# mnigm2001/Software-Defined-Radio

Hardware: AMD Instinct MI355X
Metric: I/Q MS/s through front-end FIR+decimate+demod(+audio) per job; % HBM roofline (higher is better)
Workload: dtype i8+f32

## Files before the change

### include/fmrx.h

```cpp
#ifndef FMRX_H
#define FMRX_H

#include <stddef.h>
#include <stdint.h>

#ifdef __cplusplus
extern "C" {
#endif

#if defined(__GNUC__)
#define FMRX_API __attribute__((visibility("default")))
#else
#define FMRX_API
#endif

typedef enum fmrx_status {
    FMRX_OK = 0,
    FMRX_EINVAL = 1,
    FMRX_ENODEV = 2,
    FMRX_EHIP = 3,
    FMRX_ENOMEM = 4
} fmrx_status;

FMRX_API const char *fmrx_version(void);
// ... 31 lines not shown
    size_t nseg;
    unsigned repaired;
    float max_dphase, max_dinteg;
    float tol_phase, tol_integ;
} fmrx_pll_parallel_info;
#define FMRX_PLL_RECORD_FLOATS 9
#define fmrx_pll_parallel_max_segments(n) ((size_t)(n) / 32 + 2)
FMRX_API int fmrx_fm_pll_parallel(const float *in, size_t n, float *nco_out, float *state, float freq, float Fs,
                                  float ncoScale, float phaseAdjust, float normBandwidth, double off_hint,
                                  fmrx_pll_parallel_info *info, float *records, uint64_t *mask);
FMRX_API int fmrx_stereo_mix(const float *stereo_filt, const float *pll, size_t n, float *mixer);
FMRX_API int fmrx_stereo_combine(const float *stereo_final, const float *mono, size_t n, float *left, float *right);
FMRX_API int fmrx_pcm16(const float *audio, size_t n, int16_t *out, int wrap);

FMRX_API int fmrx_deemph_design(double fs, double tau_us, float *p, float *b0);
FMRX_API int fmrx_deemph(float *y, const float *x, size_t rows, size_t n, size_t pitch, float p, float b0, float *state,
                         unsigned *missed);
FMRX_API int fmrx_deemph_dev(float *d_y, const float *d_x, size_t rows, size_t n, size_t pitch, float p, float b0, float *d_state,
                             unsigned long long *d_missed, void *stream);

FMRX_API int fmrx_diag_libm(int fn, const float *a, const float *b, size_t n, float *out);
FMRX_API int fmrx_diag_demod_fast(float *out, const float *iq, size_t n, float prev_i, float prev_q, int bounded);
FMRX_API int fmrx_diag_stream_read_dev(const void *d_buf, size_t bytes, int method, void *stream);
FMRX_API int fmrx_estimate_psd(float *freq, float *psd, const float *samples, size_t n, float Fs, int nfft);

typedef struct fmrx_params {
    int mode;
    int rf_Fs, if_Fs;
    float audio_Fs;
    int rf_decim, audio_decim, audio_upsamp;
    int rf_taps;
    int audio_taps;
    int stereo_taps;
    int block_bytes;
} fmrx_params;

FMRX_API int fmrx_mode_params(int mode, int rf_taps, int base_audio_taps, int stereo_taps, fmrx_params *p);

typedef struct fmrx_pipeline fmrx_pipeline;

#define FMRX_PCM_WRAP 1
#define FMRX_PCM_SATURATE 0

FMRX_API int fmrx_pipeline_create(fmrx_pipeline **out, const fmrx_params *p, int channels, size_t max_block_bytes,
                                  int device);
FMRX_API int fmrx_pipeline_destroy(fmrx_pipeline *pl);
// ... 366 lines not shown
```

### software-defined-radio_amd/__init__.py

```python
from __future__ import annotations

import ctypes as C
import os

import numpy as np

_HERE = os.path.dirname(os.path.abspath(__file__))
LIB_PATH = os.environ.get("FMRX_LIB") or os.path.join(_HERE, "lib", "libfmrx.so")
HEADER_PATH = os.path.join(os.path.dirname(_HERE), "include", "fmrx.h")

OK, EINVAL, ENODEV, EHIP, ENOMEM = 0, 1, 2, 3, 4
PCM_WRAP, PCM_SATURATE = 1, 0
TAPS = {"if_i": 0, "if_q": 1, "demod": 2, "mono_filt": 3, "carrier_filt": 4, "stereo_filt": 5, "pll": 6, "mixer": 7,
        "stereo_final": 8, "trig_arg": 9}


class FmrxError(RuntimeError):
    def __init__(self, code: int, msg: str):
        super().__init__(f"fmrx error {code}: {msg}")
        self.code = code


if not os.path.exists(LIB_PATH):
    raise ImportError(
# ... 216 lines not shown


def _option_value(name: str, value) -> int:
    names = _OPTION_NAMES.get(name, {})
    if isinstance(value, str) and value not in names:
        raise FmrxError(EINVAL, f"option {name}: '{value}' is not one of its named values {sorted(names)}")
    return names[value] if isinstance(value, str) else int(value)


def set_option(name: str, value) -> None:
    _check(lib.fmrx_set_option(name.encode(), _option_value(name, value)))


def get_option(name: str) -> int:
    v = C.c_long(0)
    _check(lib.fmrx_get_option(name.encode(), C.byref(v)))
    return v.value


def diagStreamRead(d_ptr, n_bytes, method=0, stream=None) -> None:
    _check(lib.fmrx_diag_stream_read_dev(d_ptr, n_bytes, method, stream))


def hostAlloc(nbytes: int, dtype=np.uint8) -> np.ndarray:
    p = _vp()
    _check(lib.fmrx_host_alloc(C.byref(p), int(nbytes)))
    buf = (C.c_uint8 * int(nbytes)).from_address(p.value)
    arr = np.frombuffer(buf, dtype=dtype)
    arr.flags.writeable = True
    _PINNED[arr.ctypes.data] = (p.value, buf)
    return arr


def hostFree(arr: np.ndarray) -> None:
    p, _ = _PINNED.pop(arr.ctypes.data)
    _check(lib.fmrx_host_free(p))


_PINNED: dict = {}


def deviceLibm(fn: str, a, b=None, flat=False) -> np.ndarray:
    a = _f32(a)
    out = np.zeros(len(a), np.float32)
    bb = _f32(b) if b is not None else None
    _check(lib.fmrx_diag_libm({"sinf": 0, "cosf": 1, "atan2f": 2}[fn] + (3 if flat else 0), a,
# ... 1185 lines not shown
```

### software-defined-radio_amd/csrc/capi.hip

```cpp
#include "fmrx_internal.hpp"
#include "rds_station.hpp"
#include <vector>

#include "build_id.hpp"

namespace fmrx {

static thread_local char g_err[512] = "";

int fail(int code, const char *fmt, ...)
{
    va_list ap;
    va_start(ap, fmt);
    vsnprintf(g_err, sizeof(g_err), fmt, ap);
    va_end(ap);
    return code;
}

int require_device()
{
    int n = 0;
    hipError_t e = hipGetDeviceCount(&n);
    if (e != hipSuccess || n <= 0) {
        (void)hipGetLastError();
// ... 502 lines not shown
    if ((!out || !iq) && n) return fail(FMRX_EINVAL, "diag_demod_fast: null buffer");
    if (bounded != 0 && bounded != 1) return fail(FMRX_EINVAL, "diag_demod_fast: bounded must be 0 or 1");
    if (n == 0) return FMRX_OK;
    FMRX_TRY(require_device());
    Stage st;
    Dev<float> dz, dp, dc;
    const float prev[2] = {prev_i, prev_q};
    FMRX_TRY(st.in(dz, iq, 2 * n));
    FMRX_TRY(st.in(dp, prev, 2));
    FMRX_TRY(st.out(dc, n));
    FMRX_TRY(k_fm_demod_if(dz.p, n, dp.p, nullptr, dc.p, bounded ? 2 : 1, nullptr));
    return st.back(out, dc);
}

int fmrx_diag_stream_read_dev(const void *d_buf, size_t bytes, int method, void *stream)
{
    if (!d_buf || method < 0 || (method & ~0x10000) > 4096) return fail(FMRX_EINVAL, "diag_stream_read_dev: bad arguments");
    FMRX_TRY(require_device());
    Dev<unsigned> sink;
    FMRX_TRY(Stage(kStreamReadSlot, 1).out(sink, 4));
    return k_stream_read(d_buf, bytes, method, sink.p, static_cast<hipStream_t>(stream));
}

int fmrx_estimate_psd(float *freq, float *psd, const float *samples, size_t n, float Fs, int nfft)
{
    if (!freq || !psd || !samples) return fail(FMRX_EINVAL, "estimate_psd: null buffer");
    if (nfft < 2 || nfft % 2 || nfft > 65536) return fail(FMRX_EINVAL, "estimate_psd: nfft must be even and in 2..65536");
    if (n < static_cast<size_t>(nfft)) return fail(FMRX_EINVAL, "estimate_psd: %zu samples < nfft %d", n, nfft);
    if (!(Fs > 0)) return fail(FMRX_EINVAL, "estimate_psd: Fs must be positive");
    FMRX_TRY(require_device());
    Stage st;
    Dev<float> a, b, c, d;
    const size_t nseg = n / nfft, half = nfft / 2;
    FMRX_TRY(st.out(a, n));
    FMRX_TRY(st.put(a.p, samples, nseg * nfft));
    FMRX_TRY(st.out(b, nseg * half));
    FMRX_TRY(st.out(c, half));
    FMRX_TRY(st.out(d, half));
    FMRX_TRY(k_estimate_psd(a.p, n, Fs, nfft, b.p, c.p, d.p, nullptr));
    FMRX_TRY(st.back(freq, c));
    return st.back(psd, d);
}

struct fmrx_fe_plan {
    FePlan plan;
};
// ... 191 lines not shown
```

### software-defined-radio_amd/csrc/fmrx_internal.hpp

```cpp
#pragma once
#include <hip/hip_runtime.h>

#include <cstdarg>
#include <cstdint>
#include <cstdio>
#include <cstdlib>
#include <cstring>
#include <mutex>
#include <string>
#include <vector>

#include "fmrx.h"

namespace fmrx {

int fail(int code, const char *fmt, ...);

#define FMRX_HIP(expr)                                                                         \
    do {                                                                                       \
        hipError_t e_ = (expr);                                                                \
        if (e_ != hipSuccess)                                                                  \
            return ::fmrx::fail(FMRX_EHIP, "%s failed: %s (%s:%d)", #expr, hipGetErrorString(e_), \
                                __FILE__, __LINE__);                                           \
    } while (0)

#define FMRX_TRY(expr)              \
    do {                            \
        int rc_ = (expr);           \
        if (rc_ != FMRX_OK) return rc_; \
    } while (0)

#define FMRX_LAUNCH_CHECK(name, ...)                                                                                              \
    do {                                                                                                                          \
        hipError_t e_ = hipGetLastError();                                                                                        \
        if (e_ != hipSuccess) return ::fmrx::fail(FMRX_EHIP, "launch " name ": %s", ##__VA_ARGS__, hipGetErrorString(e_));        \
    } while (0)

int require_device();

struct Options {
    int fe_variant = 0, tuner_variant = 0, demod = 0, overlap_calls = 0;
    long fused_min_audio = 65536;
    int resample_l2 = 0, resample_exact = 0, resample_chains = 0;
    int pll_warmup = -1, pll_segment = -1, pll_start = 1, pll_mode = 0;
    int deemph_warmup = -1, deemph_segment = -1, deemph_mode = 0;
};
Options &default_options();
std::mutex &options_mutex();
Options options_snapshot();
int set_option_in(Options &o, const char *name, long value);
int get_option_in(const Options &o, const char *name, long *value);

template <typename T>
struct DevBuf {
    T *p = nullptr;
    size_t n = 0;
    DevBuf() = default;
    DevBuf(const DevBuf &) = delete;
    DevBuf &operator=(const DevBuf &) = delete;
    ~DevBuf() { release(); }
    void release()
    {
        if (p) (void)hipFree(p);
        p = nullptr;
        n = 0;
// ... 33 lines not shown
int fe_mfma_bank_lead(const FePlan &pl);
int fe_mfma_bank_launch(const FePlan &pl, const uint8_t *d_slots, long total_bytes, long in_pitch, long block_off, int n_channels,
                        long k_lo, long k_hi, float *d_demod, long out_pitch, long out_off, hipStream_t stream);
int fe_launch(const FePlan &pl, const uint8_t *d_iq, size_t n_samples, const uint8_t *d_hist, float *d_if,
              const Options &o, hipStream_t stream, bool force_generic);
int fe_hist_bytes(int taps, int decim);
bool fe_fused_available(const FePlan &pl, const uint8_t *d_iq, size_t n_samples);
int fe_demod_launch(const FePlan &pl, const uint8_t *d_iq, size_t n_samples, const uint8_t *d_hist,
                    const float *d_prev_override, float *d_demod, float *d_if, float *d_prev_out,
                    uint8_t *d_hist_next, const Options &o, hipStream_t stream);

struct AudioPlan {
    int taps = 0, decim = 0;
    bool fast = false;
    DevBuf<float> table;
    DevBuf<float> h;
    DevBuf<float> mfma_table;
};
int audio_mfma_table_init(AudioPlan &pl, const float *h, int taps, int decim);
bool mono_fused_available(const FePlan &fe, const AudioPlan &au, const uint8_t *d_iq, size_t n_samples, const uint8_t *d_hist);
int mono_fused_launch(const FePlan &fe, const AudioPlan &au, const uint8_t *d_iq, size_t n_samples, const uint8_t *d_hist,
                      const float *d_prev, const float *d_dhist_end, float *d_demod_tail, int tail_keep, float *d_prev_out,
                      float *d_audio, int16_t *d_pcm, int wrap, uint8_t *d_hist_next, const Options &o, hipStream_t stream);
int audio_plan_init(AudioPlan &pl, const float *h, int taps, int decim);
bool audio_fast_available(const AudioPlan &pl, const float *d_x);
int audio_fir_launch(const AudioPlan &pl, const float *d_x, const float *d_hist_end, size_t n_in, int delay, float *d_y,
                     int16_t *d_pcm, int wrap, hipStream_t stream, bool force_generic);

struct ResamplePlan {
    int taps = 0, decim = 0, upsamp = 0;
    int J = 0, JP = 0;
    int span = 0;
    bool fast = false;
    int npass = 0, W = 0, span_l = 0;
    DevBuf<float> table;
    DevBuf<float> h;
    bool mfma = false;
    int mfma_ks4 = 0, mfma_ngroups = 0, mfma_pieces = 0;
    bool mfma_reach_ok = false;
    mutable int mfma_wgs_per_cu[2] = {0, 0};
    DevBuf<float> mfma_img;
    DevBuf<int> mfma_top, mfma_groups;
};
int resample_plan_init(ResamplePlan &pl, const float *h, int taps, int decim, int upsamp);
constexpr int kResampleFront = 256, kResampleBack = 1024;
int resample_launch(const ResamplePlan &pl, const float *d_x, size_t n_in, int delay, float *d_y, const Options &o,
// ... 210 lines not shown
```

### software-defined-radio_amd/csrc/kernels_fe_mfma.hip

```cpp
#include "device_math.hpp"
#include "fe_mfma_host.hpp"
#include "fmrx_internal.hpp"

#include <cmath>
#include <type_traits>
#include <utility>

namespace fmrx {
namespace {

using i4 = int __attribute__((ext_vector_type(4)));
using f2 = float __attribute__((ext_vector_type(2)));
using f4 = float __attribute__((ext_vector_type(4)));

constexpr int kNtPolicy = 2;

constexpr int iclamp(int v, int lo, int hi) { return v < lo ? lo : (v > hi ? hi : v); }
constexpr int igcd(int a, int b) { return b == 0 ? a : igcd(b, a % b); }

template <int T, int D, int PF = 0>
struct MfCfg {
    static constexpr int COL_OUT = 8;
    static constexpr int COLS = 16;
    static constexpr int TILE_OUT = COL_OUT * (COLS - 1);
    static constexpr int COL_BYTES = 2 * D * COL_OUT;
    static constexpr int STRIDE_BYTES = COL_BYTES * (COLS - 1);
    static constexpr int FRONT = (2 * (T - 1) + 15) / 16 * 16;
    static constexpr int WIN = FRONT + 2 * D * (COL_OUT - 1) + 2;
    static constexpr int KSTEPS = (WIN + 63) / 64;
    static constexpr int NDIG = kFeMfmaDigits;
    static constexpr int LEAD = COL_BYTES + FRONT;
    static constexpr int TILE_WIN = COL_BYTES * (COLS - 1) + 64 * KSTEPS;
    static constexpr int NPF = TILE_WIN / 1024;
    static constexpr int REM_LANES = (TILE_WIN % 1024) / 16;
    static constexpr int NP = NPF + (REM_LANES ? 1 : 0);
    static constexpr int SLOT = NP * 1024;
    static constexpr int P = PF ? PF : iclamp(8192 / TILE_WIN, 2, 8);
    static constexpr int NSLOT = P + 1;
    static constexpr int RING = NSLOT * SLOT;
    static_assert(TILE_WIN % 16 == 0 && COL_BYTES % 16 == 0, "16-byte fragments");
    static constexpr int YOUNGER = NP * P;
// ... 331 lines not shown
            int lo = acc[0][k];
            if (C::NDIG >= 2) lo += acc[1][k] * 256;
            const float flo = static_cast<float>(lo) * scale_lo;
            v[k] = C::NDIG >= 3 ? __builtin_fmaf(static_cast<float>(acc[2][k]), scale_hi, flo) : flo;
        }
        const float pi = __shfl(v[2], src_lane, 64), pq = __shfl(v[3], src_lane, 64);
        const float d0 = demod_fast(v[0], v[1], pi, pq), d1 = demod_fast(v[2], v[3], v[0], v[1]);
        const int c = tile / bk.tiles_per_row, j = tile - c * bk.tiles_per_row;
        const long ol = static_cast<long>(j) * C::TILE_OUT + C::COL_OUT * (col - 1) + 2 * g;
        if (col > 0 && ol < bk.n_row) *reinterpret_cast<f2 *>(demod + c * bk.out_pitch + bk.out_off + ol) = (f2){d0, d1};
        slot = slot + 1 == C::NSLOT ? 0 : slot + 1;
        fill = fill + 1 == C::NSLOT ? 0 : fill + 1;
    }
}

template <int T, int D, int TA, int DA>
struct FuCfg {
    using F = MfCfg<T, D>;
    static constexpr int TILE_OUT = 128;
    static constexpr int TILE_BYTES = F::COL_BYTES * 16;
    static constexpr int NPF = TILE_BYTES / 1024;
    static constexpr int REM_LANES = (TILE_BYTES % 1024) / 16;
    static constexpr int NP = NPF + (REM_LANES ? 1 : 0);
    static constexpr int P = iclamp(6144 / TILE_BYTES, 2, 8);
    static constexpr int NSLOT = P + 2;
    static constexpr int RING = NSLOT * TILE_BYTES;
    static constexpr int PIECE0 = NPF ? 1024 : TILE_BYTES;
    static_assert(F::WIN - F::COL_BYTES <= PIECE0, "window overlap must fit the next slot's first piece");
    static_assert(64 * F::KSTEPS - F::COL_BYTES <= RING - TILE_BYTES, "K padding laps the ring");
    static constexpr int YOUNGER = (NP - 1) + NP * P;
    static_assert(YOUNGER <= 63, "vmcnt is 6 bits");
    static constexpr int AB_OUT = 256;
    static constexpr int TB = AB_OUT * DA / TILE_OUT;
    static_assert(TB * TILE_OUT == AB_OUT * DA, "batches end on tile boundaries");
    static constexpr int SLOT_STEP = igcd(TB, NSLOT);
    static constexpr int NSTART = NSLOT / SLOT_STEP;
    static constexpr int LANE_OFF_END = F::COL_BYTES * (F::COLS - 1) + 16 * 3 + 16;
    static constexpr int AWIN = (TA - 1) + 15 * DA + 1;
    static constexpr int AK = (AWIN + 15) / 16 * 4;
    static_assert(AK % 4 == 0 && (TA - 1) % 4 == 0, "window in whole 16-byte groups");
    static constexpr int KPT = ((AK + TB - 3) / (TB - 2) + 3) / 4 * 4;
    static constexpr int NPH = (AK + KPT - 1) / KPT;
    static constexpr int DR_MIN = AB_OUT * DA + TA - 1 + (4 * AK - AWIN) + (NPH + 1) * TILE_OUT;
    static constexpr int DR = (DR_MIN + TILE_OUT - 1) / TILE_OUT * TILE_OUT;
    static_assert(NPH <= TB - 2, "a batch must be done before the next one completes");
    static_assert(AB_OUT * DA + TA - 1 + (4 * AK - AWIN) + (NPH + 1) * TILE_OUT <= DR, "ring too small for the delayed multiply");
    static_assert(DR % TILE_OUT == 0, "tiles must not wrap inside");
    static_assert(TA - 1 <= TILE_OUT - 1, "one dry tile must cover the audio history");
    static constexpr int MIRROR = 4 * KPT;
    static_assert(MIRROR <= TILE_OUT, "the mirror is refreshed by the tile at position 0");
    static constexpr int LDS_WAVE = RING + (DR + MIRROR) * 4;
};

template <class C, class F>
__device__ __forceinline__ void fu_dma_slot(const uint8_t *__restrict__ x, const uint8_t *__restrict__ hist_end, long n_bytes,
                                            int u, uint8_t *ring, int rs, int lane)
{
    dma_window<C::NPF, C::REM_LANES, kNtPolicy>(x, hist_end, n_bytes, static_cast<long>(u) * C::TILE_BYTES - F::FRONT,
                                                ring + rs * C::TILE_BYTES, lane);
}

template <int T, int D, int TA, int DA>
__global__ __launch_bounds__(256, 2) void mono_fused_kernel(
    const uint8_t *__restrict__ x, const uint8_t *__restrict__ hist_end, long n_bytes, const i4 *__restrict__ a_img,
    float scale_lo, const float *__restrict__ au_img, const float2 *__restrict__ prev_in,
    const float *__restrict__ dhist_end, float *__restrict__ demod_tail, int tail_keep, float2 *__restrict__ prev_out,
    float *__restrict__ audio, int16_t *__restrict__ pcm, int wrap, long n_out, int n_tiles, long n_audio, int n_batches,
    int batches_per_wave, uint8_t *__restrict__ hist_next, int hist_bytes)
{
    using C = FuCfg<T, D, TA, DA>;
    using F = typename C::F;
    extern __shared__ __attribute__((aligned(16))) uint8_t lds_raw[];
    const int lane = threadIdx.x & 63;
    const int wave = __builtin_amdgcn_readfirstlane(static_cast<int>(threadIdx.x >> 6));
// ... 16 lines not shown
    for (int j = 0; j < F::KSTEPS; j++)
#pragma unroll
        for (int d = 0; d < F::NDIG; d++) a[j][d] = a_img[(j * F::NDIG + d) * 64 + lane];
    float au[C::AK];
#pragma unroll
    for (int j = 0; j < C::AK; j++) au[j] = au_img[j * 64 + lane];
    float ci = 0.0f, cq = 0.0f;
    for (int i = lane; i < C::DR + C::MIRROR; i += 64) dring[i] = 0.0f;
    if (t0 == 0) {
        const float2 p = *prev_in;
        ci = p.x;
        cq = p.y;
        for (int i = lane; i < TA - 1; i += 64) dring[C::TILE_OUT - (TA - 1) + i] = dhist_end[i - (TA - 1)];
    }
    asm volatile("s_waitcnt vmcnt(0) lgkmcnt(0)" ::: "memory");
#pragma unroll
    for (int j = 0; j < F::KSTEPS; j++)
#pragma unroll
        for (int d = 0; d < F::NDIG; d++) asm volatile("" : "+v"(a[j][d]));
#pragma unroll
    for (int j = 0; j < C::AK; j++) asm volatile("" : "+v"(au[j]));
    asm volatile("" : "+v"(ci), "+v"(cq));

    for (int u = tb; u <= tb + C::P && u <= t1; u++) fu_dma_slot<C, F>(x, hist_end, n_bytes, u, ring, u % C::NSLOT, lane);

    const int col = lane & 15, g = lane >> 4;
    const int lane_off = F::COL_BYTES * col + 16 * g;
    const float scale_hi = scale_lo * 65536.0f;
    const int src_lane = lane >= 16 ? lane - 16 : lane + 47;
    int wrap_adr[F::KSTEPS];
#pragma unroll
    for (int j = 0; j < F::KSTEPS; j++) {
        const int adr = (C::NSLOT - 1) * C::TILE_BYTES + lane_off + 64 * j;
        wrap_adr[j] = adr >= C::RING ? adr - C::RING : adr;
    }
    int slot = tb % C::NSLOT, fill = (tb + C::P + 1) % C::NSLOT;
    int dpos = C::TILE_OUT;
    bool pend = false;
    int pend_ph = 0, pend_ws = 0;
    long pend_a0 = 0;
    f4 y0 = (f4){0.0f, 0.0f, 0.0f, 0.0f}, y1 = y0;
    f4 xs[C::KPT / 4];
    auto slice_load = [&]() {
#pragma unroll
        for (int k = 0; k < C::KPT / 4; k++)
            xs[k] = *reinterpret_cast<const f4 *>(dring + pend_ws + 16 * k);
        pend_ws += 4 * C::KPT;
        pend_ws = pend_ws >= C::DR ? pend_ws - C::DR : pend_ws;
    };
    auto slice_mfma = [&]() {
#pragma unroll
        for (int ph = 0; ph < C::NPH; ph++)
            if (pend_ph == ph) {
#pragma unroll
                for (int j = ph * C::KPT; j < (ph + 1) * C::KPT && j < C::AK; j++) {
                    const float xv = xs[(j - ph * C::KPT) / 4][j % 4];
                    if (j & 1) y1 = __builtin_amdgcn_mfma_f32_16x16x4f32(au[j], xv, y1, 0, 0, 0);
                    else y0 = __builtin_amdgcn_mfma_f32_16x16x4f32(au[j], xv, y0, 0, 0, 0);
                }
// ... 32 lines not shown
        int sb = (bt * C::AB_OUT * DA - (TA - 1)) - (C::TILE_OUT * tb - C::TILE_OUT);
        pend_ws = (sb + 16 * col * DA + 4 * g) % C::DR;
        y0 = (f4){0.0f, 0.0f, 0.0f, 0.0f};
        y1 = y0;
    };
    int t_fast1 = 0;
    bool fast_last = false;
    if (scale_lo >= 8.8817842e-16f) {
        const long in_x = (n_bytes - C::NP * 1024L + F::FRONT) / C::TILE_BYTES;
        const long no_tail = (n_out - tail_keep) / C::TILE_OUT - 1;
        long lim = t1 - C::P - 1;
        lim = lim < in_x - C::P - 1 ? lim : in_x - C::P - 1;
        lim = lim < no_tail ? lim : no_tail;
        t_fast1 = lim + 1 >= C::TB ? static_cast<int>((lim + 1) / C::TB) * C::TB : 0;
        fast_last = t1 % C::TB == 0 && t1 - C::TB >= t0 && t1 <= in_x && t1 - 1 <= no_tail;
    }
    int t_cur = tb;
    const long rbase = static_cast<long>(tb) * C::TILE_BYTES;
    const long reach = static_cast<long>(t1 - tb + 1) * C::TILE_BYTES + C::NP * 1024L;
    const __amdgpu_buffer_rsrc_t xr = __builtin_amdgcn_make_buffer_rsrc(
        const_cast<uint8_t *>(x + rbase), 0, static_cast<int>(reach < n_bytes - rbase ? reach : n_bytes - rbase), 0x00020000);
    const int lane16 = 16 * lane;
    const uint8_t *lring = ring + lane_off;
    auto fast_tile = [&](auto kc, auto lastc, auto sc, int t) {
        constexpr int k = decltype(kc)::value;
        constexpr int U = (decltype(sc)::value + k) % C::NSLOT;
        constexpr int FILL = (U + C::P + 1) % C::NSLOT;
        constexpr bool STEADY = !decltype(lastc)::value || k + C::P + 1 <= C::TB;
        constexpr int WAIT = STEADY ? C::YOUNGER : (C::NP - 1) + C::NP * (C::TB - k - 1);
        auto slice_k = [&]() {
#pragma unroll
            for (int j = k * C::KPT; j < (k + 1) * C::KPT && j < C::AK; j++) {
                const float xv = xs[(j - k * C::KPT) / 4][j % 4];
                if (j & 1) y1 = __builtin_amdgcn_mfma_f32_16x16x4f32(au[j], xv, y1, 0, 0, 0);
                else y0 = __builtin_amdgcn_mfma_f32_16x16x4f32(au[j], xv, y0, 0, 0, 0);
            }
        };
        if constexpr (STEADY) {
            const int soff = (t + C::P + 1 - tb) * C::TILE_BYTES - F::FRONT;
            for_each_index(std::make_integer_sequence<int, C::NP>{}, [&](auto qc) {
                constexpr int q = decltype(qc)::value;
                if (q < C::NPF || lane < C::REM_LANES)
                    __builtin_amdgcn_raw_ptr_buffer_load_lds(
                        xr, (__attribute__((address_space(3))) void *)(ring + FILL * C::TILE_BYTES + q * 1024), 16, lane16,
                        soff + q * 1024, 0, kNtPolicy);
            });
        }
        wait_vmcnt<WAIT>();
        __builtin_amdgcn_fence(__ATOMIC_ACQUIRE, "wavefront");
        __builtin_amdgcn_wave_barrier();
        i4 b[F::KSTEPS];
        for_each_index(std::make_integer_sequence<int, F::KSTEPS>{}, [&](auto jc) {
            constexpr int j = decltype(jc)::value;
            constexpr int OFF = U * C::TILE_BYTES + 64 * j;
            if constexpr (OFF + C::LANE_OFF_END > C::RING) {
                static_assert(U == C::NSLOT - 1, "only the last slot wraps");
                b[j] = *reinterpret_cast<const i4 *>(ring + wrap_adr[j]);
            } else {
                b[j] = *reinterpret_cast<const i4 *>(lring + OFF);
            }
        });
// ... 14 lines not shown
        float v[4];
#pragma unroll
        for (int q = 0; q < 4; q++) {
            int lo = acc[0][q];
            if (F::NDIG >= 2) lo += acc[1][q] * 256;
            const float flo = static_cast<float>(lo) * scale_lo;
            v[q] = F::NDIG >= 3 ? __builtin_fmaf(static_cast<float>(acc[2][q]), scale_hi, flo) : flo;
        }
        float pi = __shfl(v[2], src_lane, 64), pq = __shfl(v[3], src_lane, 64);
        pi = lane == 0 ? ci : pi;
        pq = lane == 0 ? cq : pq;
        ci = __builtin_bit_cast(float, __builtin_amdgcn_readlane(__builtin_bit_cast(int, v[2]), 63));
        cq = __builtin_bit_cast(float, __builtin_amdgcn_readlane(__builtin_bit_cast(int, v[3]), 63));
        const float d0 = demod_fast_bounded(v[0], v[1], pi, pq);
        const float d1 = demod_fast_bounded(v[2], v[3], v[0], v[1]);
        const int ol = F::COL_OUT * col + 2 * g;
        *reinterpret_cast<f2 *>(dring + dpos + ol) = (f2){d0, d1};
        if (dpos == 0 && ol < C::MIRROR) *reinterpret_cast<f2 *>(dring + C::DR + ol) = (f2){d0, d1};
        dpos = dpos + C::TILE_OUT == C::DR ? 0 : dpos + C::TILE_OUT;
        if constexpr (k < C::NPH) slice_k();
        if constexpr (k == C::NPH - 1) store_batch();
    };
    auto fast_batch = [&](auto lastc) {
        const int s0 = t_cur % C::NSLOT;
        for_each_index(std::make_integer_sequence<int, C::NSTART>{}, [&](auto ic) {
            constexpr int S = decltype(ic)::value * C::SLOT_STEP;
            if (s0 == S)
                for_each_index(std::make_integer_sequence<int, C::TB>{}, [&](auto kc) {
                    fast_tile(kc, lastc, std::integral_constant<int, S>{}, t_cur + decltype(kc)::value);
                });
        });
        begin_batch(t_cur / C::TB);
        t_cur += C::TB;
    };
    for (int &t = t_cur;;) {
        if (t >= t0 && (t < t_fast1 || (fast_last && t == t1 - C::TB)) && t % C::TB == 0 && (!pend || pend_ph == 0)) {
            if (!pend) {
                begin_batch(t / C::TB);
                pend_a0 = n_audio;
            }
            while (t < t_fast1) fast_batch(std::false_type{});
            if (fast_last && t == t1 - C::TB) fast_batch(std::true_type{});
            slot = t % C::NSLOT;
            fill = (t + C::P + 1) % C::NSLOT;
        }
        const bool have_tile = t < t1;
        bool completed = false;
        if (have_tile) {
            const bool sl = pend;
            const bool steady = t + C::P + 1 <= t1;
            if (steady) fu_dma_slot<C, F>(x, hist_end, n_bytes, t + C::P + 1, ring, fill, lane);
            if (steady) wait_vmcnt<C::YOUNGER>();
            else wait_vmcnt<0>();
            __builtin_amdgcn_fence(__ATOMIC_ACQUIRE, "wavefront");
            __builtin_amdgcn_wave_barrier();

            i4 b[F::KSTEPS];
            if (slot != C::NSLOT - 1) {
                const uint8_t *bsrc = ring + slot * C::TILE_BYTES + lane_off;
#pragma unroll
                for (int j = 0; j < F::KSTEPS; j++) b[j] = *reinterpret_cast<const i4 *>(bsrc + 64 * j);
            } else {
#pragma unroll
                for (int j = 0; j < F::KSTEPS; j++) b[j] = *reinterpret_cast<const i4 *>(ring + wrap_adr[j]);
            }
            if (sl) slice_load();
            __builtin_amdgcn_s_waitcnt(0xC07F);
// ... 41 lines not shown
            }
            slot = slot + 1 == C::NSLOT ? 0 : slot + 1;
            fill = fill + 1 == C::NSLOT ? 0 : fill + 1;
            dpos = dpos + C::TILE_OUT == C::DR ? 0 : dpos + C::TILE_OUT;
            if (sl) {
                slice_mfma();
                slice_done();
            }
            completed = t >= t0 && ((t + 1) % C::TB == 0 || t + 1 == n_tiles);
            t++;
        }

        while (pend && (completed || !have_tile)) {
            slice_load();
            slice_mfma();
            slice_done();
        }
        if (completed) begin_batch((t - 1) / C::TB);
        if (!have_tile && !pend) break;
    }
}

template <int T, int D, int TA, int DA>
int launch_fused_mono(const FePlan &fe, const AudioPlan &au, const uint8_t *d_iq, size_t n_samples, const uint8_t *d_hist,
                      const float *d_prev, const float *d_dhist_end, float *d_demod_tail, int tail_keep, float *d_prev_out,
                      float *d_audio, int16_t *d_pcm, int wrap, uint8_t *d_hist_next, hipStream_t stream)
{
    using C = FuCfg<T, D, TA, DA>;
    if (C::F::FRONT > fe.hist_bytes) return fail(FMRX_EINVAL, "mono_fused: history too short");
    const long n_out = static_cast<long>(n_samples / D);
    const long n_tiles = (n_out + C::TILE_OUT - 1) / C::TILE_OUT;
    const long n_audio = n_out / DA;
    const long n_batches = (n_audio + C::AB_OUT - 1) / C::AB_OUT;
    long wgs_per_cu = (160 * 1024) / (4L * C::LDS_WAVE);
    if (wgs_per_cu > 2) wgs_per_cu = 2;
    const int lds_bytes = 4 * C::LDS_WAVE;
    const long max_waves = 256 * wgs_per_cu * 4;
    const long bpw = (n_batches + max_waves - 1) / max_waves;
    const long grid = ((n_batches + bpw - 1) / bpw + 3) / 4;
    if (lds_bytes > 64 * 1024) {
        static bool raised[64] = {};
        int dev = 0;
        FMRX_HIP(hipGetDevice(&dev));
        if (dev < 0 || dev >= 64 || !raised[dev]) {
            FMRX_HIP(hipFuncSetAttribute(reinterpret_cast<const void *>(&mono_fused_kernel<T, D, TA, DA>),
                                         hipFuncAttributeMaxDynamicSharedMemorySize, lds_bytes));
            if (dev >= 0 && dev < 64) raised[dev] = true;
        }
    }
    hipLaunchKernelGGL((mono_fused_kernel<T, D, TA, DA>), dim3(static_cast<unsigned>(grid)), dim3(256), lds_bytes, stream,
                       d_iq, d_hist + fe.hist_bytes, static_cast<long>(2 * n_samples), reinterpret_cast<const i4 *>(fe.a_img.p),
                       fe.scale_lo, au.mfma_table.p, reinterpret_cast<const float2 *>(d_prev), d_dhist_end, d_demod_tail,
                       tail_keep, reinterpret_cast<float2 *>(d_prev_out), d_audio, d_pcm, wrap, n_out, static_cast<int>(n_tiles),
                       n_audio, static_cast<int>(n_batches), static_cast<int>(bpw), d_hist_next, fe.hist_bytes);
    FMRX_LAUNCH_CHECK("mono_fused_kernel<%d,%d,%d,%d>", T, D, TA, DA);
    return FMRX_OK;
}

#define FMRX_FUSED_CASES(X)                                                                         \
    X(101, 10, 101, 5) X(151, 10, 101, 5) X(13, 10, 101, 5) X(101, 10, 13, 5) X(151, 10, 13, 5) X(13, 10, 13, 5) \
    X(101, 5, 101, 6) X(151, 5, 101, 6) X(13, 5, 101, 6) X(101, 5, 13, 6) X(151, 5, 13, 6) X(13, 5, 13, 6)

#define FMRX_FE_MFMA_CASES(X) X(13, 10) X(101, 10) X(151, 10) X(13, 5) X(101, 5) X(151, 5) X(13, 3) X(101, 3) X(151, 3)

}

int fe_mfma_plan_init(FePlan &pl, const float *h, int taps, int decim)
{
    pl.mfma = false;
    int s = 0;
    if (!fe_mfma_scale(h, taps, kFeMfmaDigits, &s)) return FMRX_OK;
    std::vector<int8_t> img;
// ... 86 lines not shown
    return FMRX_OK;
}

bool mono_fused_available(const FePlan &fe, const AudioPlan &au, const uint8_t *d_iq, size_t n_samples, const uint8_t *d_hist)
{
    if (!fe_mfma_available(fe, d_iq, n_samples, d_hist) || !au.mfma_table.p) return false;
    for (int k = 0; k < 1; k++) {
#define X(T_, D_, TA_, DA_) \
    if (fe.taps == T_ && fe.decim == D_ && au.taps == TA_ && au.decim == DA_) return true;
        FMRX_FUSED_CASES(X)
#undef X
    }
    return false;
}

int mono_fused_launch(const FePlan &fe, const AudioPlan &au, const uint8_t *d_iq, size_t n_samples, const uint8_t *d_hist,
                      const float *d_prev, const float *d_dhist_end, float *d_demod_tail, int tail_keep, float *d_prev_out,
                      float *d_audio, int16_t *d_pcm, int wrap, uint8_t *d_hist_next, const Options &o, hipStream_t stream)
{
    if (!d_prev || !d_dhist_end) return fail(FMRX_EINVAL, "mono_fused_launch: null argument");
#define X(T_, D_, TA_, DA_)                                                                                          \
    if (fe.taps == T_ && fe.decim == D_ && au.taps == TA_ && au.decim == DA_)                                         \
        return launch_fused_mono<T_, D_, TA_, DA_>(fe, au, d_iq, n_samples, d_hist, d_prev, d_dhist_end, d_demod_tail, \
                                                   tail_keep, d_prev_out, d_audio, d_pcm, wrap, d_hist_next, stream);
    FMRX_FUSED_CASES(X)
#undef X
    return fail(FMRX_EINVAL, "mono_fused_launch: no kernel for this filter shape");
}

}
```

### software-defined-radio_amd/csrc/options.cpp

```cpp
#include "fmrx_internal.hpp"

#include <cctype>
#include <cerrno>
#include <climits>

namespace fmrx {
namespace {

struct OptionRow {
    const char *name;
    int Options::*i; long Options::*l;
    long lo, hi;
    bool not_zero;
    struct { const char *name; long value; } named[2];
};
constexpr OptionRow kOptions[] = {
    {"fe_variant", &Options::fe_variant, nullptr, 0, 1, false, {{"mfma", 0}, {"valu", 1}}},
    {"fused_min_audio", nullptr, &Options::fused_min_audio, LONG_MIN, LONG_MAX, false, {}},
    {"resample_l2", &Options::resample_l2, nullptr, INT_MIN, INT_MAX, false, {}},
    {"resample_exact", &Options::resample_exact, nullptr, INT_MIN, INT_MAX, false, {}},
    {"resample_chains", &Options::resample_chains, nullptr, INT_MIN, INT_MAX, false, {}},
    {"overlap_calls", &Options::overlap_calls, nullptr, INT_MIN, INT_MAX, false, {}},
    {"pll_warmup", &Options::pll_warmup, nullptr, INT_MIN, INT_MAX, false, {}},
    {"pll_segment", &Options::pll_segment, nullptr, INT_MIN, INT_MAX, false, {}},
    {"pll_start", &Options::pll_start, nullptr, INT_MIN, INT_MAX, false, {}},
    {"pll_mode", &Options::pll_mode, nullptr, 0, 2, false, {}},
    {"demod", &Options::demod, nullptr, 0, 1, false, {{"discriminator", 0}, {"arctan", 1}}},
    {"tuner_variant", &Options::tuner_variant, nullptr, 0, 1, false, {{"mfma", 0}, {"generic", 1}}},
    {"deemph_warmup", &Options::deemph_warmup, nullptr, -1, 1 << 20, false, {}},
    {"deemph_segment", &Options::deemph_segment, nullptr, -1, 1 << 20, true, {}},
    {"deemph_mode", &Options::deemph_mode, nullptr, 0, 1, false, {}},
};

const OptionRow *find_option(const char *name)
{
    for (const OptionRow &r : kOptions)
        if (name && std::strcmp(name, r.name) == 0) return &r;
    fail(FMRX_EINVAL, "unknown option '%s'", name ? name : "(null)");
    return nullptr;
}

// ... 71 lines not shown
```

Baseline: 2.631 million.

## Grid-aligned 1KiB input DMA schedule for decim-10 fused mono kernel

For decimation 10, the fused mono kernel now issues its LDS ring loads as fixed 1 KiB grid pieces, splitting any piece that wraps the ring, instead of tile-sized pieces. Per-tile vmcnt waits are derived by a constexpr schedule checker that proves every tile's bytes have landed. Ring slots are now indexed relative to the wave's first tile, and the prefetch depth and K-slice size per tile are fixed constants for D=10. The change aims for fewer, larger and aligned DMA loads and deeper prefetch, at the cost of heavy template complexity; it also adds a fused_max_waves option and an occupancy diagnostic.

```diff
diff --git a/include/fmrx.h b/include/fmrx.h
--- a/include/fmrx.h
+++ b/include/fmrx.h
@@ -77,6 +77,7 @@
 FMRX_API int fmrx_diag_libm(int fn, const float *a, const float *b, size_t n, float *out);
 FMRX_API int fmrx_diag_demod_fast(float *out, const float *iq, size_t n, float prev_i, float prev_q, int bounded);
 FMRX_API int fmrx_diag_stream_read_dev(const void *d_buf, size_t bytes, int method, void *stream);
+FMRX_API int fmrx_diag_fused_occupancy(int *blocks);
 FMRX_API int fmrx_estimate_psd(float *freq, float *psd, const float *samples, size_t n, float Fs, int nfft);
 
 typedef struct fmrx_params {
diff --git a/software-defined-radio_amd/__init__.py b/software-defined-radio_amd/__init__.py
--- a/software-defined-radio_amd/__init__.py
+++ b/software-defined-radio_amd/__init__.py
@@ -262,6 +262,12 @@
     _check(lib.fmrx_diag_stream_read_dev(d_ptr, n_bytes, method, stream))
 
 
+def diagFusedOccupancy() -> int:
+    n = _int(0)
+    _check(_sig("fmrx_diag_fused_occupancy", [C.POINTER(_int)])(C.byref(n)))
+    return n.value
+
+
 def hostAlloc(nbytes: int, dtype=np.uint8) -> np.ndarray:
     p = _vp()
     _check(lib.fmrx_host_alloc(C.byref(p), int(nbytes)))
diff --git a/software-defined-radio_amd/csrc/capi.hip b/software-defined-radio_amd/csrc/capi.hip
--- a/software-defined-radio_amd/csrc/capi.hip
+++ b/software-defined-radio_amd/csrc/capi.hip
@@ -548,6 +548,13 @@
     return k_stream_read(d_buf, bytes, method, sink.p, static_cast<hipStream_t>(stream));
 }
 
+int fmrx_diag_fused_occupancy(int *blocks)
+{
+    if (!blocks) return fail(FMRX_EINVAL, "diag_fused_occupancy: null result pointer");
+    FMRX_TRY(require_device());
+    return mono_fused_occupancy(blocks);
+}
+
 int fmrx_estimate_psd(float *freq, float *psd, const float *samples, size_t n, float Fs, int nfft)
 {
     if (!freq || !psd || !samples) return fail(FMRX_EINVAL, "estimate_psd: null buffer");
diff --git a/software-defined-radio_amd/csrc/fmrx_internal.hpp b/software-defined-radio_amd/csrc/fmrx_internal.hpp
--- a/software-defined-radio_amd/csrc/fmrx_internal.hpp
+++ b/software-defined-radio_amd/csrc/fmrx_internal.hpp
@@ -41,6 +41,7 @@
 struct Options {
     int fe_variant = 0, tuner_variant = 0, demod = 0, overlap_calls = 0;
     long fused_min_audio = 65536;
+    int fused_max_waves = 0;
     int resample_l2 = 0, resample_exact = 0, resample_chains = 0;
     int pll_warmup = -1, pll_segment = -1, pll_start = 1, pll_mode = 0;
     int deemph_warmup = -1, deemph_segment = -1, deemph_mode = 0;
@@ -120,6 +121,7 @@
 int mono_fused_launch(const FePlan &fe, const AudioPlan &au, const uint8_t *d_iq, size_t n_samples, const uint8_t *d_hist,
                       const float *d_prev, const float *d_dhist_end, float *d_demod_tail, int tail_keep, float *d_prev_out,
                       float *d_audio, int16_t *d_pcm, int wrap, uint8_t *d_hist_next, const Options &o, hipStream_t stream);
+int mono_fused_occupancy(int *blocks);
 int audio_plan_init(AudioPlan &pl, const float *h, int taps, int decim);
 bool audio_fast_available(const AudioPlan &pl, const float *d_x);
 int audio_fir_launch(const AudioPlan &pl, const float *d_x, const float *d_hist_end, size_t n_in, int delay, float *d_y,
diff --git a/software-defined-radio_amd/csrc/kernels_fe_mfma.hip b/software-defined-radio_amd/csrc/kernels_fe_mfma.hip
--- a/software-defined-radio_amd/csrc/kernels_fe_mfma.hip
+++ b/software-defined-radio_amd/csrc/kernels_fe_mfma.hip
@@ -16,7 +16,6 @@
 constexpr int kNtPolicy = 2;
 
 constexpr int iclamp(int v, int lo, int hi) { return v < lo ? lo : (v > hi ? hi : v); }
-constexpr int igcd(int a, int b) { return b == 0 ? a : igcd(b, a % b); }
 
 template <int T, int D, int PF = 0>
 struct MfCfg {
@@ -394,25 +393,27 @@
     static constexpr int NPF = TILE_BYTES / 1024;
     static constexpr int REM_LANES = (TILE_BYTES % 1024) / 16;
     static constexpr int NP = NPF + (REM_LANES ? 1 : 0);
-    static constexpr int P = iclamp(6144 / TILE_BYTES, 2, 8);
+    static constexpr int P = D == 10 ? 3 : iclamp(6144 / TILE_BYTES, 2, 8);
     static constexpr int NSLOT = P + 2;
     static constexpr int RING = NSLOT * TILE_BYTES;
-    static constexpr int PIECE0 = NPF ? 1024 : TILE_BYTES;
-    static_assert(F::WIN - F::COL_BYTES <= PIECE0, "window overlap must fit the next slot's first piece");
     static_assert(64 * F::KSTEPS - F::COL_BYTES <= RING - TILE_BYTES, "K padding laps the ring");
     static constexpr int YOUNGER = (NP - 1) + NP * P;
+    static_assert(F::TILE_WIN - TILE_BYTES <= (NPF ? 1024 : TILE_BYTES), "the general loop waits for one piece of the next slot");
     static_assert(YOUNGER <= 63, "vmcnt is 6 bits");
     static constexpr int AB_OUT = 256;
     static constexpr int TB = AB_OUT * DA / TILE_OUT;
     static_assert(TB * TILE_OUT == AB_OUT * DA, "batches end on tile boundaries");
-    static constexpr int SLOT_STEP = igcd(TB, NSLOT);
-    static constexpr int NSTART = NSLOT / SLOT_STEP;
+    static_assert(TB % NSLOT == 0, "a batch is a whole number of ring laps");
+    static constexpr bool GRID = D == 10;
+    static_assert(!GRID || ((TB * TILE_BYTES) % 1024 == 0 && ((P + 1) * TILE_BYTES) % 1024 == 0),
+                  "a batch, and what the general loop has fetched in front of one, end on the grid");
     static constexpr int LANE_OFF_END = F::COL_BYTES * (F::COLS - 1) + 16 * 3 + 16;
     static constexpr int AWIN = (TA - 1) + 15 * DA + 1;
     static constexpr int AK = (AWIN + 15) / 16 * 4;
     static_assert(AK % 4 == 0 && (TA - 1) % 4 == 0, "window in whole 16-byte groups");
-    static constexpr int KPT = ((AK + TB - 3) / (TB - 2) + 3) / 4 * 4;
+    static constexpr int KPT = D == 10 ? (TA > 13 ? 24 : 12) : (TA > 13 ? 8 : 4);
     static constexpr int NPH = (AK + KPT - 1) / KPT;
+    static_assert(KPT % 4 == 0, "a slice is whole groups of 4 K-steps");
     static constexpr int DR_MIN = AB_OUT * DA + TA - 1 + (4 * AK - AWIN) + (NPH + 1) * TILE_OUT;
     static constexpr int DR = (DR_MIN + TILE_OUT - 1) / TILE_OUT * TILE_OUT;
     static_assert(NPH <= TB - 2, "a batch must be done before the next one completes");
@@ -422,6 +423,127 @@
     static constexpr int MIRROR = 4 * KPT;
     static_assert(MIRROR <= TILE_OUT, "the mirror is refreshed by the tile at position 0");
     static constexpr int LDS_WAVE = RING + (DR + MIRROR) * 4;
+    static_assert(2 * 4 * LDS_WAVE <= 160 * 1024, "two workgroups per CU");
+};
+
+template <class C>
+struct FuSched {
+    using F = typename C::F;
+    static constexpr int TILE = C::TILE_BYTES, RING = C::RING, TB = C::TB;
+    static constexpr int NEED = F::COL_BYTES * (F::COLS - 1) + F::WIN;
+    static constexpr int NPIECE = TB * TILE / 1024;
+    static constexpr int LAST_PIECE = (TILE * (TB - 1) + F::TILE_WIN - 1) / 1024;
+    static constexpr int MAXI = 128;
+    struct Seq {
+        int lo[MAXI], hi[MAXI], at[MAXI], n;
+    };
+    static constexpr int grid_end(int k) { return (TILE * k + RING) / 1024; }
+    static constexpr bool piece_wraps(int j) { return 1024 * j % RING + 1024 > RING; }
+    static constexpr int wrap_head(int j) { return RING - 1024 * j % RING; }
+
+    static constexpr void push(Seq &s, int lo, int hi, int at)
+    {
+        s.lo[s.n] = lo, s.hi[s.n] = hi, s.at[s.n] = at;
+        s.n++;
+    }
+    static constexpr void push_piece(Seq &s, int j, int at)
+    {
+        if (!piece_wraps(j)) return push(s, 1024 * j, 1024 * j + 1024, at);
+        push(s, 1024 * j, 1024 * j + wrap_head(j), at);
+        push(s, 1024 * j + wrap_head(j), 1024 * j + 1024, at);
+    }
+    static constexpr void push_tile(Seq &s, int u, int at)
+    {
+        for (int q = 0; q < C::NP; q++) push(s, TILE * u + 1024 * q, q < C::NPF ? TILE * u + 1024 * q + 1024 : TILE * u + TILE, at);
+    }
+    static constexpr Seq walk(bool entry, bool last)
+    {
+        Seq s{};
+        if (entry || !C::GRID)
+            for (int u = -1; u <= C::P; u++) push_tile(s, u, -1);
+        else
+            for (int j = 0; j < grid_end(-1); j++) push_piece(s, j, -1);
+        for (int k = 0; k < TB; k++)
+            if (C::GRID) {
+                for (int j = grid_end(k - 1); j < grid_end(k); j++)
+                    if (!last || j <= LAST_PIECE) push_piece(s, j, k);
+            } else if (!last || k + C::P + 1 <= TB) {
+                push_tile(s, k + C::P + 1, k);
+            }
+        return s;
+    }
+    static constexpr int issued(const Seq &s, int k)
+    {
+        int n = 0;
+        while (n < s.n && s.at[n] <= k) n++;
+        return n;
+    }
+    static constexpr int wait_of(const Seq &s, int k)
+    {
+        int need = -1;
+        for (int i = 0; i < issued(s, k); i++)
+            if (s.lo[i] < TILE * k + NEED && s.hi[i] > TILE * k) need = i;
+        return issued(s, k) - 1 - need;
+    }
+    static constexpr int wait(bool last, int k)
+    {
+        const int a = wait_of(walk(false, last), k), b = wait_of(walk(true, last), k);
+        return a < b ? a : b;
+    }
+    static constexpr bool landed(bool entry, bool last)
+    {
+        const Seq s = walk(entry, last);
+        for (int k = 0; k < TB; k++) {
+            const int done = issued(s, k) - wait(last, k);
+            int p = TILE * k;
+            while (p < TILE * k + NEED) {
+                int q = p;
+                for (int i = 0; i < done; i++)
+                    if (s.lo[i] <= p && p < s.hi[i] && s.hi[i] > q) q = s.hi[i];
+                if (q == p) return false;
+                p = q;
+            }
+            for (int i = done; i < s.n; i++)
+                if (s.lo[i] < TILE * k + NEED && s.hi[i] > TILE * k) return false;
+        }
+        return true;
+    }
+    static constexpr bool in_time(bool entry, bool last)
+    {
+        const Seq s = walk(entry, last);
+        for (int i = 0; i < s.n; i++)
+            if (s.hi[i] - RING > TILE * s.at[i] || s.hi[i] - s.lo[i] > 1024 || s.lo[i] % 16 || s.hi[i] % 16) return false;
+        return true;
+    }
+    static constexpr bool counts_fit()
+    {
+        for (int k = 0; k < TB; k++)
+            if (wait(false, k) > 63 || wait(true, k) > 63 || wait(false, k) < 0 || wait(true, k) < 0) return false;
+        return true;
+    }
+    static constexpr bool one_wrap()
+    {
+        int n = 0;
+        for (int j = 0; j < NPIECE; j++)
+            if (piece_wraps(j) && (++n > 1 || wrap_head(j) != 512)) return false;
+        return true;
+    }
+    static constexpr bool hands_over()
+    {
+        return grid_end(TB - 1) - NPIECE == grid_end(-1) && NPIECE * 1024 == TB * TILE && TB * TILE % RING == 0 &&
+               grid_end(-1) * 1024 == (C::P + 1) * TILE;
+    }
+    static constexpr bool proved()
+    {
+        static_assert(landed(false, false) && landed(true, false), "steady batch: a tile reads bytes that its wait does not cover");
+        static_assert(landed(false, true) && landed(true, true), "last batch: a tile reads bytes that its wait does not cover");
+        static_assert(in_time(false, false) && in_time(true, false) && in_time(false, true) && in_time(true, true),
+                      "a piece is issued over bytes that are still to be read");
+        static_assert(counts_fit(), "vmcnt is 6 bits");
+        static_assert(!C::GRID || (one_wrap() && hands_over()), "the grid does not fit the ring");
+        static_assert(C::GRID || (wait(false, 0) == C::YOUNGER && wait(false, TB - 1) == C::YOUNGER), "tile-cut schedule");
+        return true;
+    }
 };
 
 template <class C, class F>
@@ -484,7 +606,8 @@
     for (int j = 0; j < C::AK; j++) asm volatile("" : "+v"(au[j]));
     asm volatile("" : "+v"(ci), "+v"(cq));
 
-    for (int u = tb; u <= tb + C::P && u <= t1; u++) fu_dma_slot<C, F>(x, hist_end, n_bytes, u, ring, u % C::NSLOT, lane);
+    for (int u = tb; u <= tb + C::P && u <= t1; u++)
+        fu_dma_slot<C, F>(x, hist_end, n_bytes, u, ring, (u - t0 + C::NSLOT) % C::NSLOT, lane);
 
     const int col = lane & 15, g = lane >> 4;
     const int lane_off = F::COL_BYTES * col + 16 * g;
@@ -496,7 +619,7 @@
         const int adr = (C::NSLOT - 1) * C::TILE_BYTES + lane_off + 64 * j;
         wrap_adr[j] = adr >= C::RING ? adr - C::RING : adr;
     }
-    int slot = tb % C::NSLOT, fill = (tb + C::P + 1) % C::NSLOT;
+    int slot = (tb - t0 + C::NSLOT) % C::NSLOT, fill = (slot + C::P + 1) % C::NSLOT;
     int dpos = C::TILE_OUT;
     bool pend = false;
     int pend_ph = 0, pend_ws = 0;
@@ -575,12 +698,15 @@
         const_cast<uint8_t *>(x + rbase), 0, static_cast<int>(reach < n_bytes - rbase ? reach : n_bytes - rbase), 0x00020000);
     const int lane16 = 16 * lane;
     const uint8_t *lring = ring + lane_off;
-    auto fast_tile = [&](auto kc, auto lastc, auto sc, int t) {
+    using S = FuSched<C>;
+    static_assert(S::proved(), "input schedule");
+    auto fast_tile = [&](auto kc, auto lastc, int t) {
         constexpr int k = decltype(kc)::value;
-        constexpr int U = (decltype(sc)::value + k) % C::NSLOT;
-        constexpr int FILL = (U + C::P + 1) % C::NSLOT;
-        constexpr bool STEADY = !decltype(lastc)::value || k + C::P + 1 <= C::TB;
-        constexpr int WAIT = STEADY ? C::YOUNGER : (C::NP - 1) + C::NP * (C::TB - k - 1);
+        constexpr int U = k % C::NSLOT;
+        [[maybe_unused]] constexpr int FILL = (U + C::P + 1) % C::NSLOT;
+        constexpr bool LAST = decltype(lastc)::value;
+        constexpr bool STEADY = !LAST || k + C::P + 1 <= C::TB;
+        constexpr int WAIT = S::wait(LAST, k);
         auto slice_k = [&]() {
 #pragma unroll
             for (int j = k * C::KPT; j < (k + 1) * C::KPT && j < C::AK; j++) {
@@ -589,7 +715,26 @@
                 else y0 = __builtin_amdgcn_mfma_f32_16x16x4f32(au[j], xv, y0, 0, 0, 0);
             }
         };
-        if constexpr (STEADY) {
+        if constexpr (C::GRID) {
+            const int sbat = (t - k - tb) * C::TILE_BYTES - F::FRONT;
+            for_each_index(std::make_integer_sequence<int, S::grid_end(k) - S::grid_end(k - 1)>{}, [&](auto qc) {
+                constexpr int j = S::grid_end(k - 1) + decltype(qc)::value;
+                constexpr int RO = 1024 * j % C::RING;
+                constexpr int HEAD = S::piece_wraps(j) ? S::wrap_head(j) : 1024;
+                if constexpr (LAST && j > S::LAST_PIECE) {
+                } else if constexpr (HEAD == 1024) {
+                    __builtin_amdgcn_raw_ptr_buffer_load_lds(xr, (__attribute__((address_space(3))) void *)(ring + RO), 16, lane16,
+                                                             sbat + 1024 * j, 0, kNtPolicy);
+                } else {
+                    if (lane < HEAD / 16) {
+                        __builtin_amdgcn_raw_ptr_buffer_load_lds(xr, (__attribute__((address_space(3))) void *)(ring + RO), 16, lane16,
+                                                                 sbat + 1024 * j, 0, kNtPolicy);
+                        __builtin_amdgcn_raw_ptr_buffer_load_lds(xr, (__attribute__((address_space(3))) void *)(ring + 0), 16, lane16,
+                                                                 sbat + (1024 * j + HEAD), 0, kNtPolicy);
+                    }
+                }
+            });
+        } else if constexpr (STEADY) {
             const int soff = (t + C::P + 1 - tb) * C::TILE_BYTES - F::FRONT;
             for_each_index(std::make_integer_sequence<int, C::NP>{}, [&](auto qc) {
                 constexpr int q = decltype(qc)::value;
@@ -650,14 +795,8 @@
         if constexpr (k == C::NPH - 1) store_batch();
     };
     auto fast_batch = [&](auto lastc) {
-        const int s0 = t_cur % C::NSLOT;
-        for_each_index(std::make_integer_sequence<int, C::NSTART>{}, [&](auto ic) {
-            constexpr int S = decltype(ic)::value * C::SLOT_STEP;
-            if (s0 == S)
-                for_each_index(std::make_integer_sequence<int, C::TB>{}, [&](auto kc) {
-                    fast_tile(kc, lastc, std::integral_constant<int, S>{}, t_cur + decltype(kc)::value);
-                });
-        });
+        for_each_index(std::make_integer_sequence<int, C::TB>{},
+                       [&](auto kc) { fast_tile(kc, lastc, t_cur + decltype(kc)::value); });
         begin_batch(t_cur / C::TB);
         t_cur += C::TB;
     };
@@ -669,8 +808,9 @@
             }
             while (t < t_fast1) fast_batch(std::false_type{});
             if (fast_last && t == t1 - C::TB) fast_batch(std::true_type{});
-            slot = t % C::NSLOT;
-            fill = (t + C::P + 1) % C::NSLOT;
+            if constexpr (C::GRID) wait_vmcnt<0>();
+            slot = 0;
+            fill = C::P + 1;
         }
         const bool have_tile = t < t1;
         bool completed = false;
@@ -758,32 +898,40 @@
 }
 
 template <int T, int D, int TA, int DA>
+int fused_mono_raise_lds()
+{
+    constexpr int lds_bytes = 4 * FuCfg<T, D, TA, DA>::LDS_WAVE;
+    if (lds_bytes <= 64 * 1024) return FMRX_OK;
+    static bool raised[64] = {};
+    int dev = 0;
+    FMRX_HIP(hipGetDevice(&dev));
+    if (dev < 0 || dev >= 64 || !raised[dev]) {
+        FMRX_HIP(hipFuncSetAttribute(reinterpret_cast<const void *>(&mono_fused_kernel<T, D, TA, DA>),
+                                     hipFuncAttributeMaxDynamicSharedMemorySize, lds_bytes));
+        if (dev >= 0 && dev < 64) raised[dev] = true;
+    }
+    return FMRX_OK;
+}
+
+template <int T, int D, int TA, int DA>
 int launch_fused_mono(const FePlan &fe, const AudioPlan &au, const uint8_t *d_iq, size_t n_samples, const uint8_t *d_hist,
                       const float *d_prev, const float *d_dhist_end, float *d_demod_tail, int tail_keep, float *d_prev_out,
-                      float *d_audio, int16_t *d_pcm, int wrap, uint8_t *d_hist_next, hipStream_t stream)
+                      float *d_audio, int16_t *d_pcm, int wrap, uint8_t *d_hist_next, const Options &o, hipStream_t stream)
 {
     using C = FuCfg<T, D, TA, DA>;
+    static_assert(FuSched<C>::proved(), "input schedule");
     if (C::F::FRONT > fe.hist_bytes) return fail(FMRX_EINVAL, "mono_fused: history too short");
     const long n_out = static_cast<long>(n_samples / D);
     const long n_tiles = (n_out + C::TILE_OUT - 1) / C::TILE_OUT;
     const long n_audio = n_out / DA;
     const long n_batches = (n_audio + C::AB_OUT - 1) / C::AB_OUT;
-    long wgs_per_cu = (160 * 1024) / (4L * C::LDS_WAVE);
-    if (wgs_per_cu > 2) wgs_per_cu = 2;
     const int lds_bytes = 4 * C::LDS_WAVE;
-    const long max_waves = 256 * wgs_per_cu * 4;
+    long max_waves = 256 * 2 * 4;
+    if (o.fused_max_waves > 0 && o.fused_max_waves < max_waves) max_waves = o.fused_max_waves;
     const long bpw = (n_batches + max_waves - 1) / max_waves;
+    if (bpw * C::TB * C::TILE_BYTES > (1L << 30)) return fail(FMRX_EINVAL, "mono_fused: %ld batches per wave are too many", bpw);
     const long grid = ((n_batches + bpw - 1) / bpw + 3) / 4;
-    if (lds_bytes > 64 * 1024) {
-        static bool raised[64] = {};
-        int dev = 0;
-        FMRX_HIP(hipGetDevice(&dev));
-        if (dev < 0 || dev >= 64 || !raised[dev]) {
-            FMRX_HIP(hipFuncSetAttribute(reinterpret_cast<const void *>(&mono_fused_kernel<T, D, TA, DA>),
-                                         hipFuncAttributeMaxDynamicSharedMemorySize, lds_bytes));
-            if (dev >= 0 && dev < 64) raised[dev] = true;
-        }
-    }
+    FMRX_TRY((fused_mono_raise_lds<T, D, TA, DA>()));
     hipLaunchKernelGGL((mono_fused_kernel<T, D, TA, DA>), dim3(static_cast<unsigned>(grid)), dim3(256), lds_bytes, stream,
                        d_iq, d_hist + fe.hist_bytes, static_cast<long>(2 * n_samples), reinterpret_cast<const i4 *>(fe.a_img.p),
                        fe.scale_lo, au.mfma_table.p, reinterpret_cast<const float2 *>(d_prev), d_dhist_end, d_demod_tail,
@@ -916,10 +1064,18 @@
 #define X(T_, D_, TA_, DA_)                                                                                          \
     if (fe.taps == T_ && fe.decim == D_ && au.taps == TA_ && au.decim == DA_)                                         \
         return launch_fused_mono<T_, D_, TA_, DA_>(fe, au, d_iq, n_samples, d_hist, d_prev, d_dhist_end, d_demod_tail, \
-                                                   tail_keep, d_prev_out, d_audio, d_pcm, wrap, d_hist_next, stream);
+                                                   tail_keep, d_prev_out, d_audio, d_pcm, wrap, d_hist_next, o, stream);
     FMRX_FUSED_CASES(X)
 #undef X
     return fail(FMRX_EINVAL, "mono_fused_launch: no kernel for this filter shape");
 }
 
-}
+int mono_fused_occupancy(int *blocks)
+{
+    using C = FuCfg<101, 10, 101, 5>;
+    FMRX_TRY((fused_mono_raise_lds<101, 10, 101, 5>()));
+    FMRX_HIP(hipOccupancyMaxActiveBlocksPerMultiprocessor(blocks, mono_fused_kernel<101, 10, 101, 5>, 256, 4 * C::LDS_WAVE));
+    return FMRX_OK;
+}
+
+}
diff --git a/software-defined-radio_amd/csrc/options.cpp b/software-defined-radio_amd/csrc/options.cpp
--- a/software-defined-radio_amd/csrc/options.cpp
+++ b/software-defined-radio_amd/csrc/options.cpp
@@ -17,6 +17,7 @@
 constexpr OptionRow kOptions[] = {
     {"fe_variant", &Options::fe_variant, nullptr, 0, 1, false, {{"mfma", 0}, {"valu", 1}}},
     {"fused_min_audio", nullptr, &Options::fused_min_audio, LONG_MIN, LONG_MAX, false, {}},
+    {"fused_max_waves", &Options::fused_max_waves, nullptr, 0, 2048, false, {}},
     {"resample_l2", &Options::resample_l2, nullptr, INT_MIN, INT_MAX, false, {}},
     {"resample_exact", &Options::resample_exact, nullptr, INT_MIN, INT_MAX, false, {}},
     {"resample_chains", &Options::resample_chains, nullptr, INT_MIN, INT_MAX, false, {}},
```

Result: no change. 2.640 million (median of 2 runs) (+0.3%).
